# gogoex/BulletProofsPlus

Hardware: AMD Instinct MI355X
Metric: aggregated range-proof verifies/sec (n=64,m=16) (higher is better)
Workload: dtype u32 (30-bit limbs of a 381-bit prime field, v_mad_u64_u32)

## Files before the change

bulletproofsplus_amd/csrc/impl_verify.hpp:

```cpp
#pragma once
#include <functional>
#include <memory>
#include <mutex>

#include "codec.hpp"
#include "combined.hpp"
#include "fixed_launch.hpp"
#include "host_util.hpp"
#include "mixed.hpp"
#include "pippenger.hpp"

enum { BPP_STAGE_FROM_WIRE = 0, BPP_STAGE_SCALARS, BPP_STAGE_FIXED_MSM, BPP_STAGE_VAR_MSM, BPP_STAGE_FINALIZE,
       BPP_NUM_STAGES };
constexpr int BPP_PROFILE_SLOTS = 64;

namespace bpp {
struct PassShape {
    VerifyShape s;
    const uint32_t* challenges;
    TranscriptState tr0;
};
}

struct bpp_verifier {
    bpp_ctx ctx;
    bpp::VerifyShape s;
    bpp::DevBuf table;
    bpp::DevBuf challenges;
    bpp::TranscriptState tr0;
    std::vector<bpp::PassShape> views;
    bpp::DevBuf view_challenges;
    size_t table_bytes = 0;
    bool check_subgroup = false;
    bool profiling = false;
    std::vector<hipEvent_t> events;
    size_t passes_recorded = 0;
    unsigned last_blocks_per_proof = 0;
    unsigned last_horner_form = 0;
    hipStream_t aux = nullptr;
    hipEvent_t ev_fork = nullptr, ev_join = nullptr;
    std::mutex aux_mu;
    ~bpp_verifier() {
        for (hipEvent_t e : events) (void)hipEventDestroy(e);
        if (ev_fork) (void)hipEventDestroy(ev_fork);
        if (ev_join) (void)hipEventDestroy(ev_join);
        if (aux) (void)hipStreamDestroy(aux);
    }
};

namespace bpp {

inline unsigned blocks_per_proof(const VerifyShape& s, size_t count) {
    const unsigned maxb = cdiv(s.NF, FIXED_BLOCK);
    size_t tpp = ((size_t)1 << 18) / (count ? count : 1);
    tpp = std::max<size_t>(FIXED_BLOCK, std::min<size_t>(tpp, s.NF));
    const unsigned b_lat = cdiv(tpp, FIXED_BLOCK);
    const unsigned b_thr = std::min<unsigned>(cdiv((size_t)32768, count ? count : 1),
                                              std::max<unsigned>(1, s.NF / (FIXED_BLOCK * 4)));
#ifdef BPP_FORCE_PER
    if (count >= 1024) return std::max(1u, std::min<unsigned>(BPP_FORCE_PER, maxb));
#endif
    return std::max(1u, std::min(std::max(b_lat, b_thr), maxb));
}

#ifndef BPP_HORNER_TREE_MAX
#define BPP_HORNER_TREE_MAX 256
#endif
constexpr size_t HORNER_TREE_MAX = BPP_HORNER_TREE_MAX;
constexpr unsigned FOLD_GROUP = 8;
constexpr unsigned FOLD_GROUP2 = 4;

struct WsLayout {
    size_t pts, bad, scalars, prep, fthread, fpart, fpart2, fpart3, vpart, vdig, vwsum, vtbl, vscr, total;
};

template <class C>
struct VerifyImpl {
    static constexpr int N = C::Fp::N;
    static constexpr int JW = jac_words<C>();
    static constexpr int WW = 2 * N + 2;
    static constexpr int PW = WW / 2;

    static WsLayout ws_layout(const VerifyShape& s, size_t count) {
        WsLayout w;
        WsCarver o;
        w.pts = o.take(count * s.NV * 2 * N * 4);
        w.bad = o.take(count * 4);
        w.scalars = o.take(count * (size_t)s.N * 32);
        w.prep = o.take(count * vs_prep_bytes<C>(s));
        w.fthread = o.take(count * blocks_per_proof(s, count) * FIXED_BLOCK * JW * 4);
        w.fpart = o.take(count * blocks_per_proof(s, count) * (FIXED_BLOCK / FOLD_GROUP) * JW * 4);
        w.fpart2 = o.take(count * blocks_per_proof(s, count) * (FIXED_BLOCK / FOLD_GROUP / FOLD_GROUP2) * JW * 4);
        w.fpart3 = o.take(count * (FIXED_BLOCK / FOLD_GROUP / FOLD_GROUP2) * JW * 4);
        w.vpart = o.take(count * JW * 4);
        w.vdig = o.take(count * s.NV * VAR_DIGIT_STRIDE);
        w.vwsum = o.take(count * var_wsums_max<C>() * JW * 4);
        w.vtbl = o.take(count * s.NV * VAR_MULTIPLES * 2 * N * 4);
        w.vscr = o.take(count * s.NV * 2 * (VAR_MULTIPLES - 1) * N * 4);
        w.total = o.total;
        return w;
    }

    static int create(const bpp_ctx& ctx, const uint64_t* gh, const uint64_t* G, const uint64_t* H, size_t n, size_t m,
                      int window_bits, bpp_verifier** out);

    static PassShape own(const bpp_verifier* v) { return PassShape{v->s, v->challenges.u32(), v->tr0}; }
    static PassShape class_shape(const bpp_verifier* v, uint32_t c) {
        return c < v->views.size() ? v->views[c] : own(v);
    }

    static int run(bpp_verifier* v, const PassShape& ps, const uint64_t* d_points, const uint64_t* d_scalars, size_t count,
                   const uint64_t* d_challenges, uint32_t* d_ok, void* d_workspace, size_t workspace_bytes,
                   uint64_t* d_out_scalars, uint64_t* d_out_result, hipStream_t st);
    static int run(bpp_verifier* v, const uint64_t* d_points, const uint64_t* d_scalars, size_t count,
                   const uint64_t* d_challenges, uint32_t* d_ok, void* d_workspace, size_t workspace_bytes,
                   uint64_t* d_out_scalars, uint64_t* d_out_result, hipStream_t st) {
        return run(v, own(v), d_points, d_scalars, count, d_challenges, d_ok, d_workspace, workspace_bytes, d_out_scalars,
                   d_out_result, st);
    }

    static int range_scalars(const PassShape& ps, const uint64_t* d_scalars, const uint64_t* d_challenges, uint32_t* w_sc,
                             size_t count, uint32_t* w_prep, hipStream_t st) {
        const uint32_t* ch = d_challenges ? reinterpret_cast<const uint32_t*>(d_challenges) : ps.challenges;
        const uint32_t ch_stride = d_challenges ? (3 + ps.s.k) * 8 : 0;
        return launch_verify_scalars<C>(ps.s, reinterpret_cast<const uint32_t*>(d_scalars), ch, ch_stride, w_sc, count, w_prep, st);
    }

    using ScalarStage = std::function<int(uint32_t* w_sc, uint32_t* w_prep, uint32_t* w_bad, hipStream_t st)>;
    static int run_stage(bpp_verifier* v, const VerifyShape& s, const uint64_t* d_points, size_t count,
                         const ScalarStage& scalars, uint32_t* d_ok, void* d_workspace, size_t workspace_bytes,
                         uint64_t* d_out_scalars, uint64_t* d_out_result, hipStream_t st);

    static uint32_t horner_form(const VerifyShape& s, size_t count) {
        const bool small_job = (double)count * ((double)s.NF * fixed_adds_per_generator(s) / 7.0e9 + 9.2e-8) < 2.0e-3;
        return count <= HORNER_TREE_MAX ? 1u : (small_job ? 2u : 0u);
    }
    static int fork_tables(bpp_verifier* v, hipStream_t st, const uint32_t* w_pts, uint32_t* w_vt, uint32_t* w_vscr, size_t items,
                           std::unique_lock<std::mutex>& lock) {
        lock = std::unique_lock<std::mutex>(v->aux_mu);
        if (!v->aux) {
            HIPCHK(hipStreamCreateWithFlags(&v->aux, hipStreamNonBlocking));
            HIPCHK(hipEventCreateWithFlags(&v->ev_fork, hipEventDisableTiming));
            HIPCHK(hipEventCreateWithFlags(&v->ev_join, hipEventDisableTiming));
        }
        HIPCHK(hipEventRecord(v->ev_fork, st));
        HIPCHK(hipStreamWaitEvent(v->aux, v->ev_fork, 0));
        hipLaunchKernelGGL(k_var_tables<C>, dim3(cdiv(items, VAR_BLOCK)), dim3(VAR_BLOCK), 0, v->aux, w_pts, w_vt, w_vscr, items);
        HIPCHK(hipEventRecord(v->ev_join, v->aux));
        return BPP_OK;
    }
    static int join_tables(bpp_verifier* v, hipStream_t st, std::unique_lock<std::mutex>& lock) {
        HIPCHK(hipStreamWaitEvent(st, v->ev_join, 0));
        lock.unlock();
        return BPP_OK;
    }
    static hipError_t mark(hipEvent_t* ev, int idx, hipStream_t st) { return ev ? hipEventRecord(ev[idx], st) : hipSuccess; }
    template <class Layout>
    static int begin_pass(bpp_verifier* v, const PassShape& ps, const uint64_t* d_points, const uint64_t* d_scalars,
                          size_t count, const uint64_t* d_challenges, uint8_t* ws, const Layout& L, uint32_t* w_sc,
                          std::unique_lock<std::mutex>& aux_lock, hipStream_t st, hipEvent_t* ev);
    template <class Layout>
    static int begin_points(bpp_verifier* v, const VerifyShape& s, const uint64_t* d_points, size_t count, uint8_t* ws,
                            const Layout& L, std::unique_lock<std::mutex>& aux_lock, hipStream_t st, hipEvent_t* ev);
    template <class Layout, class FixedSums>
    static int weighted_windows(bpp_verifier* v, const PassShape& ps, uint8_t* ws, const Layout& L, size_t count,
                                const uint8_t* weight_key, uint64_t index_base, const uint64_t* d_weights, uint32_t per,
                                uint32_t split, std::unique_lock<std::mutex>& aux_lock, hipStream_t st,
                                FixedSums&& fixed_sums);
    template <class Layout>
    static int weighted_middle(bpp_verifier* v, const PassShape& ps, uint8_t* ws, const Layout& L, size_t count, uint32_t per,
                               uint32_t split, std::unique_lock<std::mutex>& aux_lock, hipStream_t st);
    static size_t fold_windows(const uint32_t* in, size_t nrem, uint32_t step, uint32_t* out, uint32_t per, hipStream_t st);
    static int finish(bpp_verifier* v, const VerifyShape& s, uint8_t* ws, const WsLayout& L, size_t count,
                      const uint32_t* w_sc, const uint32_t* w_vw, const uint32_t* w_bad, uint32_t* d_ok,
                      uint32_t* d_out_result, uint32_t tree, bool lone, hipStream_t st, hipEvent_t* ev);

    static int derive_challenges(bpp_verifier* v, const PassShape& ps, const uint64_t* d_points, size_t count,
                                 uint64_t* d_challenges, hipStream_t st);
    static int derive_challenges(bpp_verifier* v, const uint64_t* d_points, size_t count, uint64_t* d_challenges,
                                 hipStream_t st) {
        return derive_challenges(v, own(v), d_points, count, d_challenges, st);
    }

    struct MixedFront {
        size_t idx, pts, sc3, status, challenges, ok;
    };
    static MixedFront carve_front(WsCarver& o, const MixedPlan& p, size_t count, bool serialized) {
        MixedFront f;
        f.idx = o.take(count * (serialized ? (size_t)SX_WORDS : (size_t)MX_WORDS) * 4);
        f.pts = o.take(p.points * WW * 4);
        f.sc3 = o.take(count * 96);
        f.status = o.take(serialized ? count * 4 : 0);
        f.challenges = o.take(p.chals * 32);
        f.ok = o.take(count * 4);
        return f;
    }
    static int gather_front(const MixedPlan& p, const MixedFront& front, size_t count, const uint64_t* d_points,
                            const uint64_t* d_scalars, const uint64_t* d_challenges, uint8_t* ws, hipStream_t st);
    static int decode_front(const MixedPlan& p, const MixedFront& front, size_t count, const uint8_t* d_proofs,
                            const uint8_t* d_commitments, uint32_t version, uint8_t* ws, hipStream_t st);
    static int scatter_verdicts(const MixedFront& front, uint8_t* ws, uint32_t* d_ok, size_t count, hipStream_t st);
    struct ClassView {
        uint32_t c;
        PassShape ps;
        size_t first, count;
        uint64_t *pts, *sc3, *challenges;
    };
    template <class F>
    static int for_each_class(const bpp_verifier* v, const MixedPlan& p, const MixedFront& front, uint8_t* ws, F&& f) {
        auto U64 = [&](size_t off) { return reinterpret_cast<uint64_t*>(ws + off); };
        for (uint32_t c = 0; c < MIXED_CLASSES; c++) {
            if (!p.count[c]) continue;
            const int rc = f(ClassView{c, class_shape(v, c), p.first[c], p.count[c], U64(front.pts) + p.pt[c] * PW,
                                       U64(front.sc3) + p.first[c] * 12, U64(front.challenges) + p.chal[c] * 4});
            if (rc) return rc;
        }
// ... 324 lines not shown
        const uint32_t f1 = std::min<uint32_t>(s.NF, f0 + slab);
        const size_t total = (size_t)(f1 - f0) * runs_f;
        hipLaunchKernelGGL(k_tbl_fill<C>, dim3(cdiv(total, 64)), dim3(64), 0, nullptr, s, v->table.u32(),
                           tbl_scratch.u32(), f0, f1);
    }
    tr_initial_state<C>(s.n, s.m, reinterpret_cast<const uint32_t*>(fixed.data()), s.NF, v->tr0.st);
    std::vector<uint32_t> ch;
    default_challenges(s, ch);
    e = v->challenges.alloc(ch.size() * 4);
    if (e == hipSuccess) e = hipMemcpy(v->challenges.p, ch.data(), ch.size() * 4, hipMemcpyHostToDevice);
    std::vector<uint32_t> vch;
    std::vector<size_t> voff;
    for (uint32_t mp = 1; mp < s.m; mp <<= 1) {
        PassShape ps{};
        rc = make_verify_shape<C>(n, mp, window_bits, ps.s);
        if (rc) return rc;
        ps.s.hgap = s.n * (s.m - mp);
        std::vector<uint64_t> prefix((size_t)ps.s.NF * PW);
        std::memcpy(prefix.data(), fixed.data(), (size_t)(2 + ps.s.mn) * PW * 8);
        std::memcpy(prefix.data() + (size_t)(2 + ps.s.mn) * PW, fixed.data() + (size_t)(2 + s.mn) * PW,
                    (size_t)ps.s.mn * PW * 8);
        tr_initial_state<C>(ps.s.n, ps.s.m, reinterpret_cast<const uint32_t*>(prefix.data()), ps.s.NF, ps.tr0.st);
        std::vector<uint32_t> c1;
        default_challenges(ps.s, c1);
        voff.push_back(vch.size());
        vch.insert(vch.end(), c1.begin(), c1.end());
        v->views.push_back(ps);
    }
    if (e == hipSuccess && !vch.empty()) {
        e = v->view_challenges.alloc(vch.size() * 4);
        if (e == hipSuccess) e = hipMemcpy(v->view_challenges.p, vch.data(), vch.size() * 4, hipMemcpyHostToDevice);
        for (size_t i = 0; i < v->views.size(); i++) v->views[i].challenges = v->view_challenges.u32() + voff[i];
    }
    if (e == hipSuccess) e = hipDeviceSynchronize();
    if (e == hipSuccess) e = hipGetLastError();
    if (e != hipSuccess) return fail(BPP_E_HIP, "table build failed: ", hipGetErrorString(e));
    *out = v.release();
    return BPP_OK;
}

template <class C>
template <class Layout>
int VerifyImpl<C>::begin_points(bpp_verifier* v, const VerifyShape& s, const uint64_t* d_points, size_t count, uint8_t* ws,
                                const Layout& L, std::unique_lock<std::mutex>& aux_lock, hipStream_t st, hipEvent_t* ev) {
    uint32_t* w_pts = reinterpret_cast<uint32_t*>(ws + L.pts);
    uint32_t* w_bad = reinterpret_cast<uint32_t*>(ws + L.bad);
    const size_t npts = count * s.NV;
    HIPCHK(zero_words_async(w_bad, count * 4, st));
    HIPCHK(mark(ev, 2 * BPP_STAGE_FROM_WIRE, st));
    hipLaunchKernelGGL(k_points_from_wire<C>, dim3(cdiv(npts, 128)), dim3(128), 0, st,
                       reinterpret_cast<const uint32_t*>(d_points), w_pts, w_bad, npts, s.NV, v->check_subgroup ? 1u : 0u);
    HIPCHK(mark(ev, 2 * BPP_STAGE_FROM_WIRE + 1, st));
    return fork_tables(v, st, w_pts, reinterpret_cast<uint32_t*>(ws + L.vtbl), reinterpret_cast<uint32_t*>(ws + L.vscr), npts,
                       aux_lock);
}

template <class C>
template <class Layout>
int VerifyImpl<C>::begin_pass(bpp_verifier* v, const PassShape& ps, const uint64_t* d_points, const uint64_t* d_scalars,
                              size_t count, const uint64_t* d_challenges, uint8_t* ws, const Layout& L, uint32_t* w_sc,
                              std::unique_lock<std::mutex>& aux_lock, hipStream_t st, hipEvent_t* ev) {
    int rc = begin_points(v, ps.s, d_points, count, ws, L, aux_lock, st, ev);
    if (rc) return rc;
    HIPCHK(mark(ev, 2 * BPP_STAGE_SCALARS, st));
    rc = range_scalars(ps, d_scalars, d_challenges, w_sc, count, reinterpret_cast<uint32_t*>(ws + L.prep), st);
    if (rc) return rc;
    HIPCHK(mark(ev, 2 * BPP_STAGE_SCALARS + 1, st));
    return BPP_OK;
}

template <class C>
template <class Layout, class FixedSums>
int VerifyImpl<C>::weighted_windows(bpp_verifier* v, const PassShape& ps, uint8_t* ws, const Layout& L, size_t count,
                                    const uint8_t* weight_key, uint64_t index_base, const uint64_t* d_weights, uint32_t per,
                                    uint32_t split, std::unique_lock<std::mutex>& aux_lock, hipStream_t st,
                                    FixedSums&& fixed_sums) {
    uint32_t* w_wt = reinterpret_cast<uint32_t*>(ws + L.weights);
    WeightKey wk;
    load_key_words(d_weights ? nullptr : weight_key, wk.w);
    hipLaunchKernelGGL(k_comb_weights<C>, dim3(cdiv(count, 256)), dim3(256), 0, st, wk, index_base,
                       reinterpret_cast<const uint32_t*>(d_weights), w_wt, count);
    fixed_sums(w_wt);
    return weighted_middle(v, ps, ws, L, count, per, split, aux_lock, st);
}

template <class C>
template <class Layout>
int VerifyImpl<C>::weighted_middle(bpp_verifier* v, const PassShape& ps, uint8_t* ws, const Layout& L, size_t count,
                                   uint32_t per, uint32_t split, std::unique_lock<std::mutex>& aux_lock, hipStream_t st) {
    const VerifyShape& s = ps.s;
    auto W = [&](size_t off) { return reinterpret_cast<uint32_t*>(ws + off); };
    uint32_t *w_sc = W(L.scalars), *w_wt = W(L.weights), *w_vs = W(L.var_sc);
    uint8_t* w_vd = ws + L.vdig;
    const size_t items = count * s.NV;
    hipLaunchKernelGGL(k_comb_var_scalars<C>, dim3(cdiv(items, 256)), dim3(256), 0, st, s, w_sc, w_wt, w_vs, items);
    hipLaunchKernelGGL(k_var_digits<C>, dim3(cdiv(items, 256)), dim3(256), 0, st, s, w_vs, w_vd, items, 1u);
    int rc = join_tables(v, st, aux_lock);
    if (rc) return rc;
    const size_t vlanes = count * per;
    hipLaunchKernelGGL(k_var_windows<C>, dim3(cdiv(vlanes, VAR_BLOCK)), dim3(VAR_BLOCK), 0, st, s, w_vd, W(L.vtbl),
                       W(L.vwsum), vlanes, split, 1u);
    return BPP_OK;
}

template <class C>
size_t VerifyImpl<C>::fold_windows(const uint32_t* in, size_t nrem, uint32_t step, uint32_t* out, uint32_t per,
                                   hipStream_t st) {
    const size_t outn = cdiv(nrem, step);
    hipLaunchKernelGGL(k_comb_window_fold<C>, dim3(cdiv(outn * per, 64)), dim3(64), 0, st, in, nrem, step, out, outn * per,
                       per);
    return outn;
}

template <class C>
int VerifyImpl<C>::run(bpp_verifier* v, const PassShape& ps, const uint64_t* d_points, const uint64_t* d_scalars,
                       size_t count, const uint64_t* d_challenges, uint32_t* d_ok, void* d_workspace,
                       size_t workspace_bytes, uint64_t* d_out_scalars, uint64_t* d_out_result, hipStream_t st) {
    return run_stage(v, ps.s, d_points, count,
                     [&](uint32_t* w_sc, uint32_t* w_prep, uint32_t*, hipStream_t st_) {
                         return range_scalars(ps, d_scalars, d_challenges, w_sc, count, w_prep, st_);
                     },
                     d_ok, d_workspace, workspace_bytes, d_out_scalars, d_out_result, st);
}

template <class C>
int VerifyImpl<C>::run_stage(bpp_verifier* v, const VerifyShape& s, const uint64_t* d_points, size_t count,
                             const ScalarStage& scalars, uint32_t* d_ok, void* d_workspace, size_t workspace_bytes,
                             uint64_t* d_out_scalars, uint64_t* d_out_result, hipStream_t st) {
    const WsLayout L = ws_layout(s, count);
    if (workspace_bytes < L.total) return fail(BPP_E_ARG, "workspace too small");
    uint8_t* ws = static_cast<uint8_t*>(d_workspace);
    uint32_t* w_bad = reinterpret_cast<uint32_t*>(ws + L.bad);
    uint32_t* w_sc = d_out_scalars ? reinterpret_cast<uint32_t*>(d_out_scalars)
                                   : reinterpret_cast<uint32_t*>(ws + L.scalars);
    uint32_t* w_vt = reinterpret_cast<uint32_t*>(ws + L.vtbl);
    const unsigned bpp_ = blocks_per_proof(s, count);
    const size_t npts = count * s.NV;
    hipEvent_t* ev = nullptr;
    if (v->profiling) {
        ev = v->events.data() + (v->passes_recorded % BPP_PROFILE_SLOTS) * (BPP_NUM_STAGES * 2);
        v->passes_recorded++;
    }
    v->last_blocks_per_proof = bpp_;
    std::unique_lock<std::mutex> aux_lock;
    int rc = begin_points(v, s, d_points, count, ws, L, aux_lock, st, ev);
    if (rc) return rc;
    HIPCHK(mark(ev, 2 * BPP_STAGE_SCALARS, st));
    rc = scalars(w_sc, reinterpret_cast<uint32_t*>(ws + L.prep), w_bad, st);
    if (rc) return rc;
    HIPCHK(mark(ev, 2 * BPP_STAGE_SCALARS + 1, st));
    uint8_t* w_vd = ws + L.vdig;
    uint32_t* w_vw = reinterpret_cast<uint32_t*>(ws + L.vwsum);
    const uint32_t tree = horner_form(s, count);
    const bool lone = tree == 1 && count * bpp_ <= 1024;
    const uint32_t vgroups = lone ? VAR_GROUPS : 1u;
    v->last_horner_form = lone ? 3u : tree;
    const size_t vlanes = count * (tree == 1 ? var_wsums<C>() * vgroups : var_windows<C>());
    HIPCHK(mark(ev, 2 * BPP_STAGE_VAR_MSM, st));
    hipLaunchKernelGGL(k_var_digits<C>, dim3(cdiv(npts, 256)), dim3(256), 0, st, s, w_sc, w_vd, npts, 0u);
    rc = join_tables(v, st, aux_lock);
    if (rc) return rc;
    hipLaunchKernelGGL(k_var_windows<C>, dim3(cdiv(vlanes, VAR_BLOCK)), dim3(VAR_BLOCK), 0, st, s, w_vd, w_vt, w_vw,
                       vlanes, tree == 1 ? 1u : 0u, vgroups);
    HIPCHK(mark(ev, 2 * BPP_STAGE_VAR_MSM + 1, st));
    return finish(v, s, ws, L, count, w_sc, w_vw, w_bad, d_ok, reinterpret_cast<uint32_t*>(d_out_result), tree, lone, st,
                  ev);
}

template <class C>
int VerifyImpl<C>::finish(bpp_verifier* v, const VerifyShape& s, uint8_t* ws, const WsLayout& L, size_t count,
                          const uint32_t* w_sc, const uint32_t* w_vw, const uint32_t* w_bad, uint32_t* d_ok,
                          uint32_t* d_out_result, uint32_t tree, bool lone, hipStream_t st, hipEvent_t* ev) {
    const unsigned bpp_ = blocks_per_proof(s, count);
    uint32_t* w_fp = reinterpret_cast<uint32_t*>(ws + L.fpart);
    uint32_t* w_vp = reinterpret_cast<uint32_t*>(ws + L.vpart);
    HIPCHK(mark(ev, 2 * BPP_STAGE_FIXED_MSM, st));
    const unsigned hb = tree == 1 ? (unsigned)count : cdiv(count, tree == 2 ? FIXED_BLOCK / 8 : FIXED_BLOCK);
    uint32_t* w_ft = reinterpret_cast<uint32_t*>(ws + L.fthread);
    launch_fixed_msm<C, 0>((unsigned)(hb + count * bpp_), st, s, w_sc, v->table.u32(), w_ft, bpp_, hb, w_vw, w_vp, count,
                           lone ? 3u : tree, VpSel{1u, 0u, 1u, 0u});
    HIPCHK(mark(ev, 2 * BPP_STAGE_FIXED_MSM + 1, st));
    HIPCHK(mark(ev, 2 * BPP_STAGE_FINALIZE, st));
    const unsigned folded = bpp_ * (FIXED_BLOCK / FOLD_GROUP);
    const unsigned folded2 = folded / FOLD_GROUP2;
    uint32_t* w_fp2 = reinterpret_cast<uint32_t*>(ws + L.fpart2);
    if (tree == 1) {
        if (!lone)
            hipLaunchKernelGGL(k_partials_fold<C>, dim3(cdiv(count * folded, 64)), dim3(64), 0, st, w_ft, FOLD_GROUP, w_fp,
                               count * folded);
        hipLaunchKernelGGL(k_finalize_tree<C>, dim3((unsigned)count), dim3(64), 0, st, lone ? w_ft : w_fp,
                           lone ? bpp_ : folded, w_vp, w_bad, d_ok, d_out_result, count);
        HIPCHK(mark(ev, 2 * BPP_STAGE_FINALIZE + 1, st));
        HIPCHK(hipGetLastError());
        return BPP_OK;
    }
    hipLaunchKernelGGL(k_partials_fold<C>, dim3(cdiv(count * folded, 64)), dim3(64), 0, st, w_ft, FOLD_GROUP, w_fp,
                       count * folded);
    hipLaunchKernelGGL(k_partials_fold<C>, dim3(cdiv(count * folded2, 64)), dim3(64), 0, st, w_fp, FOLD_GROUP2, w_fp2,
                       count * folded2);
    const uint32_t* w_last = w_fp2;
    unsigned last = folded2;
    if (bpp_ > 1) {
        uint32_t* w_fp3 = reinterpret_cast<uint32_t*>(ws + L.fpart3);
        last = folded2 / bpp_;
        hipLaunchKernelGGL(k_partials_fold<C>, dim3(cdiv(count * last, 64)), dim3(64), 0, st, w_fp2, bpp_, w_fp3,
                           count * last);
        w_last = w_fp3;
    }
    hipLaunchKernelGGL(k_finalize<C>, dim3(cdiv(count, 64)), dim3(64), 0, st, w_last, last, w_vp, 1u, w_bad, d_ok,
                       d_out_result, count);
    HIPCHK(mark(ev, 2 * BPP_STAGE_FINALIZE + 1, st));
    HIPCHK(hipGetLastError());
    return BPP_OK;
}

template <class C>
int VerifyImpl<C>::run_serialized(bpp_verifier* v, const uint8_t* d_proofs, const uint8_t* d_commitments, size_t count,
                                  bool transcript, uint32_t* d_ok, void* d_workspace, size_t workspace_bytes,
                                  hipStream_t st, uint32_t version, const GroupedArgs* grouped) {
    const VerifyShape& s = v->s;
    if (int rc = container_args_ok(v, version)) return rc;
    const SerLayout L = ser_layout(s, count, grouped ? grouped->group : 0u);
    if (workspace_bytes < L.total) return fail(BPP_E_ARG, "workspace too small");
    uint8_t* ws = static_cast<uint8_t*>(d_workspace);
    uint32_t* w_rec = reinterpret_cast<uint32_t*>(ws + L.records);
    uint32_t* w_sc = reinterpret_cast<uint32_t*>(ws + L.scalars);
    uint32_t* w_st = reinterpret_cast<uint32_t*>(ws + L.status);
    uint64_t* w_ch = reinterpret_cast<uint64_t*>(ws + L.challenges);
    HIPCHK(zero_words_async(w_st, count * 4, st));
    hipLaunchKernelGGL(k_container_decode<C>, dim3(cdiv(count * s.NV, 64)), dim3(64), 0, st, s, d_proofs, d_commitments,
                       w_rec, w_sc, w_st, count, version);
    if constexpr (C::ID == 0)
        hipLaunchKernelGGL(k_records_subgroup<C>, dim3(cdiv(count * s.NV, 64)), dim3(64), 0, st, w_rec, w_st, s.NV,
                           count * s.NV);
    HIPCHK(hipGetLastError());
    if (transcript) {
        int rc = derive_challenges(v, reinterpret_cast<const uint64_t*>(w_rec), count, w_ch, st);
        if (rc) return rc;
    }
    int rc = grouped ? run_grouped(v, reinterpret_cast<const uint64_t*>(w_rec), reinterpret_cast<const uint64_t*>(w_sc), count,
                                   transcript ? w_ch : nullptr, grouped->weight_key, grouped->index_base, grouped->d_weights,
                                   grouped->group, d_ok, grouped->h_stats, ws + L.run, workspace_bytes - L.run, st)
                     : run(v, reinterpret_cast<const uint64_t*>(w_rec), reinterpret_cast<const uint64_t*>(w_sc), count,
                           transcript ? w_ch : nullptr, d_ok, ws + L.run, workspace_bytes - L.run, nullptr, nullptr, st);
    if (rc) return rc;
    hipLaunchKernelGGL(k_container_status<C>, dim3(cdiv(count, 256)), dim3(256), 0, st, w_st, d_ok, count);
    HIPCHK(hipGetLastError());
    return BPP_OK;
}

template <class C>
int VerifyImpl<C>::derive_challenges(bpp_verifier* v, const PassShape& ps, const uint64_t* d_points, size_t count,
                                     uint64_t* d_challenges, hipStream_t st) {
    (void)v;
    hipLaunchKernelGGL(k_transcript_challenges<C>, dim3(cdiv(count, 64)), dim3(64), 0, st, ps.s, ps.tr0,
                       reinterpret_cast<const uint32_t*>(d_points), reinterpret_cast<uint32_t*>(d_challenges), count);
    HIPCHK(hipGetLastError());
    return BPP_OK;
}

template <class C>
int VerifyImpl<C>::gather_front(const MixedPlan& p, const MixedFront& front, size_t count, const uint64_t* d_points,
                                const uint64_t* d_scalars, const uint64_t* d_challenges, uint8_t* ws, hipStream_t st) {
    auto U64 = [&](size_t off) { return reinterpret_cast<uint64_t*>(ws + off); };
    uint32_t* w_idx = reinterpret_cast<uint32_t*>(ws + front.idx);
    HIPCHK(hipMemcpyAsync(w_idx, p.idx.data(), p.idx.size() * 4, hipMemcpyHostToDevice, st));
    hipLaunchKernelGGL(k_mixed_gather<C>, dim3((unsigned)count), dim3(MIXED_BLOCK), 0, st, w_idx, count, d_points, d_scalars,
                       d_challenges, U64(front.pts), U64(front.sc3), U64(front.challenges));
    HIPCHK(hipGetLastError());
    return BPP_OK;
}

template <class C>
int VerifyImpl<C>::decode_front(const MixedPlan& p, const MixedFront& front, size_t count, const uint8_t* d_proofs,
                                const uint8_t* d_commitments, uint32_t version, uint8_t* ws, hipStream_t st) {
    auto W = [&](size_t off) { return reinterpret_cast<uint32_t*>(ws + off); };
    uint32_t *w_idx = W(front.idx), *w_rec = W(front.pts), *w_st = W(front.status);
    HIPCHK(hipMemcpyAsync(w_idx, p.sidx.data(), p.sidx.size() * 4, hipMemcpyHostToDevice, st));
    HIPCHK(zero_words_async(w_st, count * 4, st));
    const unsigned waves = (unsigned)(p.lanes / SER_WAVE);
    hipLaunchKernelGGL(k_container_decode_mixed<C>, dim3(waves), dim3(SER_WAVE), 0, st, p.classes, w_idx, d_proofs,
                       d_commitments, w_rec, W(front.sc3), w_st, version);
    if constexpr (C::ID == 0)
        hipLaunchKernelGGL(k_records_subgroup_mixed<C>, dim3(waves), dim3(SER_WAVE), 0, st, p.classes, w_rec, w_st);
    HIPCHK(hipGetLastError());
    return BPP_OK;
}

template <class C>
int VerifyImpl<C>::scatter_verdicts(const MixedFront& front, uint8_t* ws, uint32_t* d_ok, size_t count, hipStream_t st) {
    auto W = [&](size_t off) { return reinterpret_cast<const uint32_t*>(ws + off); };
    hipLaunchKernelGGL(k_mixed_status_scatter<C>, dim3(cdiv(count, 256)), dim3(256), 0, st, W(front.idx), W(front.status),
                       W(front.ok), d_ok, count);
    HIPCHK(hipGetLastError());
    return BPP_OK;
}

template <class C>
int VerifyImpl<C>::run_mixed(bpp_verifier* v, const uint64_t* d_points, const uint64_t* d_scalars, const uint32_t* m_of,
                             size_t count, const uint64_t* d_challenges, uint32_t* d_ok, void* d_workspace,
                             size_t workspace_bytes, uint64_t* d_out_result, hipStream_t st) {
    MixedPlan p;
    int rc = mixed_plan(v->s, m_of, count, true, p);
    if (rc) return rc;
    const MixedLayout L = mixed_layout(v, p, count);
    if (workspace_bytes < L.total) return fail(BPP_E_ARG, "workspace too small");
    uint8_t* ws = static_cast<uint8_t*>(d_workspace);
    rc = gather_front(p, L.f, count, d_points, d_scalars, d_challenges, ws, st);
    if (rc) return rc;
    uint32_t* w_ok = reinterpret_cast<uint32_t*>(ws + L.f.ok);
    uint64_t* w_res = d_out_result ? reinterpret_cast<uint64_t*>(ws + L.result) : nullptr;
    rc = for_each_class(v, p, L.f, ws, [&](const ClassView& cv) {
        return run(v, cv.ps, cv.pts, cv.sc3, cv.count, d_challenges ? cv.challenges : nullptr, w_ok + cv.first, ws + L.run,
                   workspace_bytes - L.run, nullptr, w_res ? w_res + cv.first * PW : nullptr, st);
    });
    if (rc) return rc;
    hipLaunchKernelGGL(k_mixed_scatter<C>, dim3(cdiv(count, 4)), dim3(256), 0, st,
                       reinterpret_cast<const uint32_t*>(ws + L.f.idx), count, w_ok, w_res, nullptr, d_ok, d_out_result,
                       nullptr);
    HIPCHK(hipGetLastError());
    return BPP_OK;
}

template <class C>
int VerifyImpl<C>::derive_challenges_mixed(bpp_verifier* v, const uint64_t* d_points, const uint32_t* m_of, size_t count,
                                           uint64_t* d_challenges, void* d_workspace, size_t workspace_bytes,
                                           hipStream_t st) {
    MixedPlan p;
    int rc = mixed_plan(v->s, m_of, count, true, p);
    if (rc) return rc;
    const MixedLayout L = mixed_layout(v, p, count);
    if (workspace_bytes < L.total) return fail(BPP_E_ARG, "workspace too small");
    uint8_t* ws = static_cast<uint8_t*>(d_workspace);
    rc = gather_front(p, L.f, count, d_points, nullptr, nullptr, ws, st);
    if (rc) return rc;
    rc = for_each_class(v, p, L.f, ws, [&](const ClassView& cv) {
        return derive_challenges(v, cv.ps, cv.pts, cv.count, cv.challenges, st);
    });
    if (rc) return rc;
    hipLaunchKernelGGL(k_mixed_scatter<C>, dim3(cdiv(count, 4)), dim3(256), 0, st,
                       reinterpret_cast<const uint32_t*>(ws + L.f.idx), count, nullptr, nullptr,
                       reinterpret_cast<uint64_t*>(ws + L.f.challenges), nullptr, nullptr, d_challenges);
    HIPCHK(hipGetLastError());
    return BPP_OK;
}

template <class C>
int VerifyImpl<C>::run_serialized_mixed(bpp_verifier* v, const uint8_t* d_proofs, const uint8_t* d_commitments,
                                        const uint32_t* m_of, size_t count, bool transcript, uint32_t* d_ok,
                                        void* d_workspace, size_t workspace_bytes, hipStream_t st, uint32_t version) {
    if (int rc = container_args_ok(v, version)) return rc;
    MixedPlan p;
    int rc = mixed_plan_serialized(v->s, m_of, count, (size_t)container_point_bytes<C>(version), true, p);
    if (rc) return rc;
    const SerMixedLayout L = ser_mixed_layout(v, p, count);
    if (workspace_bytes < L.total) return fail(BPP_E_ARG, "workspace too small");
    uint8_t* ws = static_cast<uint8_t*>(d_workspace);
    auto W = [&](size_t off) { return reinterpret_cast<uint32_t*>(ws + off); };
    rc = decode_front(p, L.f, count, d_proofs, d_commitments, version, ws, st);
// ... 389 lines not shown
```

bulletproofsplus_amd/csrc/kernels.hpp:

```cpp
#pragma once
#include <hip/hip_runtime.h>
#include "ec.hpp"
#include "fixed_glv.hpp"
#include "ed25519.hpp"
#include "ristretto.hpp"
#include "transcript.hpp"

namespace bpp {

constexpr unsigned MSM_BLOCK = 64;
constexpr unsigned VS_PB = 8;
constexpr unsigned VS_BLOCK = VS_PB * 64;
constexpr unsigned FIXED_BLOCK = 128;
constexpr unsigned VAR_BLOCK = 64;
template <class C>
constexpr bool var_glv() {
    return curve_has_glv<C>();
}
template <class C>
constexpr uint32_t var_windows() {
    return var_glv<C>() ? 33u : 65u;
}
template <class C>
constexpr uint32_t var_wsums() {
    return var_windows<C>() * (var_glv<C>() ? 2u : 1u);
}
constexpr uint32_t VAR_GROUPS = 3;
template <class C>
constexpr uint32_t var_wsums_max() {
    return var_wsums<C>() * VAR_GROUPS;
}
constexpr uint32_t VAR_DIGIT_STRIDE = 80;
constexpr uint32_t VAR_MULTIPLES = 8;
#ifndef BPP_FIXED_WAVES
#define BPP_FIXED_WAVES 2
#endif
#ifndef BPP_VAR_WAVES
#define BPP_VAR_WAVES 2
#endif
#ifndef BPP_VAR_TABLES_WAVES
#define BPP_VAR_TABLES_WAVES 2
#endif


static __global__ void __launch_bounds__(256) k_zero_words(uint32_t* __restrict__ p, size_t words) {
    const size_t i = (size_t)blockIdx.x * blockDim.x + threadIdx.x;
    if (i < words) p[i] = 0;
}
inline hipError_t zero_words_async(void* p, size_t bytes, hipStream_t st) {
    const size_t words = (bytes + 3) / 4;
    if (words == 0) return hipSuccess;
    hipLaunchKernelGGL(k_zero_words, dim3((unsigned)((words + 255) / 256)), dim3(256), 0, st, static_cast<uint32_t*>(p), words);
    return hipGetLastError();
}

template <int NW>
__device__ __forceinline__ void ld_words(const uint32_t* __restrict__ p, uint32_t* dst) {
    static_assert(NW % 4 == 0, "16-byte granules");
    const uint4* q = reinterpret_cast<const uint4*>(p);
#pragma unroll
    for (int i = 0; i < NW / 4; i++) {
        uint4 v = q[i];
        dst[4 * i] = v.x;
        dst[4 * i + 1] = v.y;
        dst[4 * i + 2] = v.z;
        dst[4 * i + 3] = v.w;
    }
}
template <int NW>
__device__ __forceinline__ void st_words(uint32_t* __restrict__ p, const uint32_t* src) {
    static_assert(NW % 4 == 0, "16-byte granules");
    uint4* q = reinterpret_cast<uint4*>(p);
#pragma unroll
    for (int i = 0; i < NW / 4; i++) q[i] = make_uint4(src[4 * i], src[4 * i + 1], src[4 * i + 2], src[4 * i + 3]);
}

template <class C>
__device__ __forceinline__ Aff<C> aff_ldg(const uint32_t* __restrict__ p) {
    constexpr int N = C::Fp::N;
    constexpr int JW = jac_words<C>();
    uint32_t w[2 * N];
    ld_words<2 * N>(p, w);
    return aff_load<C>(w);
}
template <class C>
__device__ __forceinline__ void aff_stg(uint32_t* __restrict__ p, const Aff<C>& a) {
    constexpr int N = C::Fp::N;
    constexpr int JW = jac_words<C>();
    uint32_t w[2 * N];
    aff_store(a, w);
    st_words<2 * N>(p, w);
}
template <class C>
__device__ __forceinline__ Jac<C> jac_ldg(const uint32_t* __restrict__ p) {
    constexpr int N = C::Fp::N;
    constexpr int JW = jac_words<C>();
    uint32_t w[JW];
    ld_words<JW>(p, w);
    return jac_load<C>(w);
}
template <class C>
__device__ __forceinline__ void jac_stg(uint32_t* __restrict__ p, const Jac<C>& a) {
    constexpr int N = C::Fp::N;
    constexpr int JW = jac_words<C>();
    uint32_t w[JW];
    jac_store(a, w);
    st_words<JW>(p, w);
}

template <class C>
__device__ __forceinline__ Jac<C> block_reduce_jac(Jac<C> acc, uint32_t* lds) {
    constexpr int N = C::Fp::N;
    constexpr int JW = jac_words<C>();
    const int tid = threadIdx.x;
    for (int half = blockDim.x >> 1; half >= 1; half >>= 1) {
        if (tid >= half && tid < 2 * half) jac_store(acc, lds + (size_t)tid * JW);
        __syncthreads();
        if (tid < half) acc = jac_add(acc, jac_load<C>(lds + (size_t)(tid + half) * JW));
        __syncthreads();
    }
    return acc;
}

template <class T>
__device__ __forceinline__ T wave_shfl(const T& v, int src_lane) {
    static_assert(sizeof(T) % 4 == 0, "whole words");
    struct Words {
        uint32_t w[sizeof(T) / 4];
    };
    Words a = __builtin_bit_cast(Words, v);
#pragma unroll
    for (int i = 0; i < (int)(sizeof(T) / 4); i++) a.w[i] = (uint32_t)__shfl((int)a.w[i], src_lane, 64);
    return __builtin_bit_cast(T, a);
}

template <class C>
__device__ __forceinline__ Jac<C> wave_sum_jac(Jac<C> x, int span = 64) {
    const int lane = threadIdx.x & 63;
#pragma unroll 1
    for (int d = span >> 1; d >= 1; d >>= 1) {
        const Jac<C> o = wave_shfl(x, lane ^ d);
        x = jac_add(x, o);
    }
    return x;
}

template <class C>
__device__ __forceinline__ Jac<C> jac_dbl_tri(const Jac<C>& p) {
    using F = Fe<typename C::Fp>;
    static_assert(C::ID != 2, "short-Weierstrass curves");
    const int lane = threadIdx.x & 63;
    const int role = lane % 3, g0 = lane - role;
    auto pick = [](bool c, const F& a, const F& b) {
        F r;
#pragma unroll
        for (int i = 0; i < C::Fp::NL; i++) r.l[i] = c ? a.l[i] : b.l[i];
        return r;
    };
    const F m1 = fe_mul(pick(role == 0, p.X, p.Y), pick(role == 0, p.X, pick(role == 1, p.Y, p.Z)));
    const F B = wave_shfl(m1, (g0 + 1) & 63);
    const F m2 = fe_sqr(pick(role == 0, fe_add(fe_dbl(m1), m1), pick(role == 1, m1, fe_add(p.X, B))));
    const F A = wave_shfl(m1, g0), Fq = wave_shfl(m2, g0), Cc = wave_shfl(m2, (g0 + 1) & 63);
    const F t = wave_shfl(m2, (g0 + 2) & 63), YZ = wave_shfl(m1, (g0 + 2) & 63);
    const F D = fe_dbl(fe_sub(fe_sub(t, A), Cc));
    const F E = fe_add(fe_dbl(A), A);
    Jac<C> r;
// ... 563 lines not shown
        j++;
    }
    const uint32_t d0 = r * TBL_RUN + 1;
    const uint32_t n = min(TBL_RUN, cnt - (d0 - 1));
    uint32_t* win = table + ((size_t)f * s.per_f + s.went[j]) * 2 * N;
    const Aff<C> base = aff_ldg<C>(win);
    Jac<C> J;
    if (d0 == 1) {
        J = jac_from_aff(base);
    } else {
        uint32_t kw[1] = {d0};
        J = aff_mul_words(base, kw, 1);
    }
    affine_chain<C>(J, win, n, win + (size_t)(d0 - 1) * 2 * N, scratch + idx * 2 * TBL_RUN * N);
}


template <class C, bool SPLIT>
__device__ __forceinline__ Jac<C> var_wsum_ld(const uint32_t* __restrict__ wsum, size_t b, uint32_t j, uint32_t groups = 1) {
    constexpr int JW = jac_words<C>();
    constexpr uint32_t NW = var_windows<C>();
    const uint32_t parts = SPLIT ? (var_wsums<C>() / NW) * groups : 1u;
    const uint32_t* W = wsum + b * parts * NW * JW;
    Jac<C> sj = jac_ldg<C>(W + (size_t)j * JW);
    for (uint32_t t = 1; t < parts; t++) sj = jac_add(sj, jac_ldg<C>(W + (size_t)(t * NW + j) * JW));
    return sj;
}

template <class C>
__device__ __forceinline__ void var_horner_lane(const uint32_t* __restrict__ wsum, uint32_t* __restrict__ out, size_t b) {
    constexpr int JW = jac_words<C>();
    constexpr uint32_t NW = var_windows<C>();
    Jac<C> acc = var_wsum_ld<C, false>(wsum, b, NW - 1);
    for (int j = (int)NW - 2; j >= 0; j--) {
        if (!acc.is_inf()) {
            acc = jac_dbl(acc);
            acc = jac_dbl(acc);
            acc = jac_dbl(acc);
            acc = jac_dbl(acc);
        }
        acc = jac_add(acc, var_wsum_ld<C, false>(wsum, b, (uint32_t)j));
    }
    jac_stg<C>(out + b * JW, acc);
}

template <class C>
__device__ __forceinline__ void var_horner_wave2(const uint32_t* __restrict__ wsum, uint32_t* __restrict__ out, size_t b,
                                                 uint32_t* lds, uint32_t groups) {
    constexpr uint32_t NW = var_windows<C>(), PER = 21;
    static_assert(NW <= 2 * PER, "two waves hold the windows");
    constexpr int JW = jac_words<C>();
    const uint32_t wave = threadIdx.x >> 6, lane = threadIdx.x & 63u;
    const uint32_t q = lane / 3, j = wave * PER + q;
    const bool has = q < PER && j < NW;
    Jac<C> R = has ? var_wsum_ld<C, true>(wsum, b, j, groups) : jac_inf<C>();
    const uint32_t times = has ? 4 * j : 0u;
    const uint32_t maxt = 4 * (wave == 0 ? PER - 1 : NW - 1);
    for (uint32_t t = 0; t < maxt; t++) {
        const Jac<C> d = jac_dbl_tri<C>(R);
        if (t < times) R = d;
    }
    R = wave_shfl(R, (int)((3 * lane) & 63u));
    if (lane >= PER || wave * PER + lane >= NW) R = jac_inf<C>();
    R = wave_sum_jac<C>(R, 32);
    if (wave == 1 && lane == 0) jac_store(R, lds);
    __syncthreads();
    if (wave == 0 && lane == 0) jac_stg<C>(out + b * JW, jac_add(R, jac_load<C>(lds)));
}

__device__ __forceinline__ void var_horner_wave_ed(const uint32_t* __restrict__ wsum, uint32_t* __restrict__ out, size_t b,
                                                   uint32_t groups) {
    using C = Ed25519;
    constexpr uint32_t NW = var_windows<C>();
    static_assert(NW == 65, "sixteen quads x four windows + one");
    constexpr int JW = jac_words<C>();
    const uint32_t lane = threadIdx.x & 63u, q = lane >> 2;
    Jac<C> acc = jac_inf<C>();
    if (q == 0) {
        acc = var_wsum_ld<C, true>(wsum, b, 64, groups);
        for (int t = 0; t < 64; t++) acc = ed_dbl_quad(acc);
    }
    for (int w = 3; w >= 0; w--) {
        acc = jac_add(acc, var_wsum_ld<C, true>(wsum, b, q + 16 * (uint32_t)w, groups));
        const int times = w > 0 ? 64 : 60;
        for (int t = 0; t < times; t++) {
            const Jac<C> d = ed_dbl_quad(acc);
            if (w > 0 || (uint32_t)t < 4 * q) acc = d;
        }
    }
    acc = wave_shfl(acc, (int)((4 * lane) & 63u));
    if (lane >= 16) acc = jac_inf<C>();
    acc = wave_sum_jac<C>(acc, 16);
    if (lane == 0) jac_stg<C>(out + b * JW, acc);
}

template <class C>
__device__ __forceinline__ void var_horner_group(const uint32_t* __restrict__ wsum, uint32_t* __restrict__ out, size_t b,
                                                 bool active, uint32_t* lds_wave) {
    constexpr uint32_t NW = var_windows<C>(), L = NW - 1, G = 8, CW = L / G;
    static_assert(L % G == 0, "windows split evenly over the eight lanes");
    constexpr int JW = jac_words<C>();
    const uint32_t lane = threadIdx.x & 63u, g = lane & (G - 1);
    Jac<C> acc = jac_inf<C>();
    if (active) {
        const int lo = (int)(g * CW);
        const int top = g == G - 1 ? (int)L : lo + (int)CW - 1;
        acc = var_wsum_ld<C, false>(wsum, b, (uint32_t)top);
        for (int j = top - 1; j >= lo; j--) {
            if (!acc.is_inf()) {
                acc = jac_dbl(acc);
                acc = jac_dbl(acc);
                acc = jac_dbl(acc);
                acc = jac_dbl(acc);
            }
            acc = jac_add(acc, var_wsum_ld<C, false>(wsum, b, (uint32_t)j));
        }
    }
    for (uint32_t stride = 1; stride < G; stride <<= 1) {
        jac_store(acc, lds_wave + (size_t)lane * JW);
        __builtin_amdgcn_fence(__ATOMIC_SEQ_CST, "wavefront");
        __builtin_amdgcn_wave_barrier();
        if (active && (g & (2 * stride - 1)) == 0) {
            Jac<C> hi = jac_load<C>(lds_wave + (size_t)(lane + stride) * JW);
            if (!hi.is_inf())
                for (uint32_t t = 0; t < 4 * CW * stride; t++) hi = jac_dbl(hi);
            acc = jac_add(acc, hi);
        }
        __builtin_amdgcn_fence(__ATOMIC_SEQ_CST, "wavefront");
        __builtin_amdgcn_wave_barrier();
    }
    if (active && g == 0) jac_stg<C>(out + b * JW, acc);
}

__device__ __forceinline__ void glds16(const uint32_t* gsrc, uint32_t lds_byte_addr) {
    unsigned keep;
    lds_byte_addr = __builtin_amdgcn_readfirstlane(lds_byte_addr);
    asm volatile("s_mov_b32 %0, m0\n\ts_mov_b32 m0, %2\n\ts_nop 0\n\tglobal_load_lds_dwordx4 %1, off\n\ts_mov_b32 m0, %0"
                 : "=&s"(keep)
                 : "v"(gsrc), "s"(lds_byte_addr)
                 : "memory");
}

#ifndef BPP_FIXED_RING
#define BPP_FIXED_RING 2
#endif
constexpr int FIXED_RING = BPP_FIXED_RING;
template <class C>
constexpr unsigned fixed_lds_bytes() {
    return (FIXED_BLOCK / 64) * (FIXED_RING * (2 * C::Fp::N / 4) + 2) * 1024;
}

struct VpSel {
    uint32_t nvp, first, cnt, prover;
};

template <class C>
constexpr int fixed_waves() {
    return C::Fp::NL > 9 ? BPP_FIXED_WAVES : 3;
}
template <class C, int ROLE = 0>
__global__ void __launch_bounds__(FIXED_BLOCK, fixed_waves<C>()) k_fixed_msm(VerifyShape s, const uint32_t* __restrict__ scalars,
                            const uint32_t* __restrict__ table, uint32_t* __restrict__ partials, uint32_t per,
                            uint32_t horner_blocks, const uint32_t* __restrict__ wsum, uint32_t* __restrict__ var_out,
                            size_t horner_count, uint32_t horner_tree, VpSel sel) {
    constexpr int N = C::Fp::N;
    constexpr int JW = jac_words<C>();
    constexpr int CH = 2 * N / 4;
    constexpr int WAVE_WORDS = (FIXED_RING * CH + 2) * 256;
    constexpr bool GLV = fixed_glv<C>();
    constexpr int NWD = GLV ? GLV_HALF_WORDS : WIN_FULL_WORDS;
    extern __shared__ __align__(16) uint32_t lds[];
    if (blockIdx.x < horner_blocks) {
        if (horner_tree == 2) {
            const size_t b = (size_t)blockIdx.x * (blockDim.x / 8) + threadIdx.x / 8;
            var_horner_group<C>(wsum, var_out, b, b < horner_count, lds + (size_t)(threadIdx.x >> 6) * 64 * JW);
        } else if (horner_tree) {
            const size_t b = blockIdx.x;
            if constexpr (var_glv<C>()) {
                if (b < horner_count) var_horner_wave2<C>(wsum, var_out, b, lds, horner_tree == 3 ? VAR_GROUPS : 1u);
            } else {
                if (b < horner_count && threadIdx.x < 64) var_horner_wave_ed(wsum, var_out, b, horner_tree == 3 ? VAR_GROUPS : 1u);
            }
        } else {
            const size_t lane = (size_t)blockIdx.x * blockDim.x + threadIdx.x;
            if (lane < horner_count) var_horner_lane<C>(wsum, var_out, lane);
        }
        return;
    }
#ifdef BPP_XCD_REMAP
    uint32_t bid = blockIdx.x - horner_blocks;
    {
        const uint32_t nb = gridDim.x - horner_blocks;
        if (nb % 8 == 0 && horner_blocks % 8 == 0) bid = (bid % 8) * (nb / 8) + bid / 8;
    }
#else
    const uint32_t bid = blockIdx.x - horner_blocks;
#endif
    const size_t b = bid / per;
    const uint32_t part = bid % per;
    const uint32_t* sc = scalars + ((b / sel.cnt) * sel.nvp + sel.first + b % sel.cnt) * (size_t)s.N * 8;
    const uint32_t stride = per * blockDim.x;
    const uint32_t lane = threadIdx.x & 63u;
    uint32_t* ring = lds + (threadIdx.x >> 6) * WAVE_WORDS;
    uint32_t* sbuf = ring + FIXED_RING * CH * 256;
    const uint32_t ring_addr = (uint32_t)reinterpret_cast<uintptr_t>(ring);
    const uint32_t sbuf_addr = ring_addr + FIXED_RING * CH * 1024;
    const uint32_t f0 = part * blockDim.x + threadIdx.x;
    const uint32_t first = part * blockDim.x;
    uint32_t NFc = s.NF, cmode = 0, cbit = 0, neg_from = 0xffffffffu;
    if (sel.prover) {
        const uint32_t vp = sel.first + (uint32_t)(b % sel.cnt);
        if (vp == 0) {
            neg_from = 2 + s.mn;
        } else if (vp <= 2 * s.k) {
            cmode = 1 + ((vp - 1) & 1u);
            cbit = s.k - 1 - (vp - 1) / 2;
            NFc = 2 + s.mn;
        } else if (vp >= 2 * s.k + 3) {
            NFc = 2;
        }
    }
    auto gen_of = [&](uint32_t x) -> uint32_t {
        if (cmode == 0 || x < 2) return x;
        uint32_t u = x - 2;
        const uint32_t hm = s.mn >> 1;
        const bool isH = u >= hm;
        if (isH) u -= hm;
        const uint32_t bitv = ((cmode == 1) != isH) ? 1u : 0u;
        const uint32_t j = ((u >> cbit) << (cbit + 1)) | (bitv << cbit) | (u & ((1u << cbit) - 1u));
        return 2 + (isH ? s.mn : 0u) + j;
    };
    const bool spread = NFc >= stride;
    const uint32_t G = spread ? NFc / stride : (first < NFc ? 1u : 0u);
    const uint32_t T = G * s.W;
    constexpr uint32_t PH = GLV ? 2u : 1u;
    const uint32_t LWH = spread ? (NFc - G * stride) * s.W : 0u;
    const uint32_t LW = PH * LWH;
    const uint32_t TT = T + (LW + stride - 1) / stride;
    const uint32_t NQ = PH * G;
    Xyzz<C> acc = xyzz_inf<C>();

    auto dma_scalar = [&](uint32_t g) {
        const uint32_t x = f0 + g * stride;
        const uint32_t* src = x < NFc ? sc + (size_t)fixed_term_index(s, gen_of(x)) * 8 : sc;
        asm volatile("s_waitcnt lgkmcnt(0)" ::: "memory");
        glds16(src, sbuf_addr);
        glds16(src + 4, sbuf_addr + 1024);
    };
    uint32_t w[NWD];
    uint32_t hneg = 0;
    uint32_t pi = 0;
    auto take = [&](const uint32_t* v, uint32_t which, uint32_t* out, uint32_t& negate) {
        if constexpr (GLV) {
            uint32_t k1[4], k2[4];
            bool n1, n2;
            glv_split_balanced<C>(v, k1, k2, n1, n2);
            win_biased<NWD>(which ? k1 : k2, s.bias, out);
            negate = which ? (n1 ? 1u : 0u) : (n2 ? 0u : 1u);
        } else {
            win_biased<NWD>(v, s.bias, out);
            negate = 0;
        }
    };
    auto take_scalar = [&]() {
        const uint4* q = reinterpret_cast<const uint4*>(sbuf);
        const uint4 lo = q[lane], hi = q[64 + lane];
        const uint32_t v[8] = {lo.x, lo.y, lo.z, lo.w, hi.x, hi.y, hi.z, hi.w};
        take(v, pi, w, hneg);
    };
    auto window = [&](uint32_t j, uint32_t& cj, uint32_t& e0) {
        if constexpr (GLV) {
            cj = win_width(s, j);
            e0 = s.went[j];
        } else {
            cj = j + 1 < s.W ? s.c : 0u;
            e0 = j << (s.c - 1);
        }
    };
    uint32_t ti = 0, gi = 0, ji = 0;
    uint32_t vbits = 0, nbits = 0;
    uint32_t bbits = 0;
    auto issue = [&]() {
        const uint32_t slot = (GLV ? pi * T + ti : ti) % FIXED_RING;
        const uint32_t* src = table;
        uint32_t valid = 0, neg = 0, viabeta = 0;
        auto entry = [&](int32_t dg, uint32_t f, uint32_t e0, uint32_t hn) {
            const uint32_t mag = dg < 0 ? (uint32_t)(-dg) : (uint32_t)dg;
            src = table + ((size_t)table_generator(s, f) * s.per_f + e0 + (mag - 1)) * 2 * N;
            valid = 1;
            neg = (dg < 0 ? 1u : 0u) ^ hn ^ (f >= neg_from ? 1u : 0u);
        };
        if (ti < T) {
            const uint32_t qi = pi * G + gi;
            if (ji == 0 && qi > 0) {
                take_scalar();
                if (qi + 1 < NQ) dma_scalar(gi + 1 < G ? gi + 1 : 0u);
            }
            const uint32_t x = f0 + gi * stride;
            uint32_t cj, e0;
            window(ji, cj, e0);
            const int32_t dg = win_next_digit(w, cj);
            if (x < NFc && dg != 0) entry(dg, gen_of(x), e0, hneg);
        } else if (pi + 1 == PH && ti < TT) {
            const uint32_t x = (ti - T) * stride + f0;
            if (x < LW) {
                const uint32_t which = x >= LWH ? 1u : 0u, xh = x - which * LWH;
                const uint32_t l = xh / s.W, jx = xh - l * s.W;
                const uint32_t f = gen_of(G * stride + l);
                uint32_t v[8], we[NWD], hn;
                ld_words<8>(sc + (size_t)fixed_term_index(s, f) * 8, v);
                take(v, which, we, hn);
                if constexpr (GLV) viabeta = 1u - which;
                int32_t dg = 0;
                uint32_t e0 = 0;
                for (uint32_t r = 0; r < s.W; r++) {
                    uint32_t cr, er;
                    window(r, cr, er);
                    const int32_t d = win_next_digit(we, cr);
                    if (r == jx) {
                        dg = d;
                        e0 = er;
                    }
                }
                if (dg != 0) entry(dg, f, e0, hn);
            }
        }
        asm volatile("s_waitcnt lgkmcnt(0)" ::: "memory");
#pragma unroll
        for (int k = 0; k < CH; k++) glds16(src + 4 * k, ring_addr + (slot * CH + k) * 1024);
        vbits = (vbits & ~(1u << slot)) | (valid << slot);
        nbits = (nbits & ~(1u << slot)) | (neg << slot);
        if constexpr (GLV) bbits = (bbits & ~(1u << slot)) | (viabeta << slot);
        ti++;
        if (++ji == s.W) {
            ji = 0;
            gi++;
        }
        if constexpr (GLV) {
            if (ti == T && pi == 0) {
                pi = 1;
                ti = 0;
                gi = 0;
                ji = 0;
            }
        }
    };
    if (G) {
        dma_scalar(0);
        asm volatile("s_waitcnt vmcnt(0)" ::: "memory");
        take_scalar();
        if (NQ > 1) dma_scalar(G > 1 ? 1u : 0u);
    }
    for (int d = 0; d < FIXED_RING; d++) issue();
// ... 231 lines not shown
```

Measured before the change: 202,100.

## Split fixed-base MSM into single-block long proofs plus multi-block tail proofs

Result: faster. 206,200 (median of 6 runs) (+2.1%).

```diff
diff --git a/bulletproofsplus_amd/csrc/fixed_plan.hpp b/bulletproofsplus_amd/csrc/fixed_plan.hpp
--- /dev/null
+++ b/bulletproofsplus_amd/csrc/fixed_plan.hpp
@@ -0,0 +1,60 @@
+#pragma once
+#include <stddef.h>
+#include <stdint.h>
+
+#include <algorithm>
+
+#include "field.hpp"
+
+namespace bpp {
+
+constexpr unsigned FIXED_BLOCK = 128;
+
+constexpr size_t FIXED_RESIDENT = 1024;
+#ifndef BPP_FIXED_SHORT_PROOFS
+#define BPP_FIXED_SHORT_PROOFS FIXED_RESIDENT
+#endif
+
+inline unsigned blocks_per_proof(uint32_t NF, size_t count) {
+    const unsigned maxb = (NF + FIXED_BLOCK - 1) / FIXED_BLOCK;
+    size_t tpp = ((size_t)1 << 18) / (count ? count : 1);
+    tpp = std::max<size_t>(FIXED_BLOCK, std::min<size_t>(tpp, NF));
+    const unsigned b_lat = (unsigned)((tpp + FIXED_BLOCK - 1) / FIXED_BLOCK);
+    const unsigned b_thr = std::min<unsigned>((unsigned)((32 * FIXED_RESIDENT + (count ? count : 1) - 1) / (count ? count : 1)),
+                                              std::max<unsigned>(1, NF / (FIXED_BLOCK * 4)));
+#ifdef BPP_FORCE_PER
+    if (count >= FIXED_RESIDENT) return std::max(1u, std::min<unsigned>(BPP_FORCE_PER, maxb));
+#endif
+    return std::max(1u, std::min(std::max(b_lat, b_thr), maxb));
+}
+
+struct FixedPlan {
+    unsigned per;
+    size_t long_count;
+};
+
+inline FixedPlan fixed_plan(uint32_t NF, size_t count, uint32_t horner_form) {
+    FixedPlan p{blocks_per_proof(NF, count), 0};
+    const size_t short_proofs = (size_t)(BPP_FIXED_SHORT_PROOFS);
+    if (horner_form == 0 && count > FIXED_RESIDENT && count > short_proofs && NF / (FIXED_BLOCK * 4) >= 2 && p.per >= 2)
+        p.long_count = count - short_proofs;
+    return p;
+}
+
+inline size_t fixed_plan_blocks(const FixedPlan& p, size_t count) { return p.long_count + (count - p.long_count) * p.per; }
+
+BPP_HD void fixed_block_of(uint32_t bid, uint32_t per, uint32_t long_count, uint32_t& proof, uint32_t& part,
+                           uint32_t& per_here) {
+    if (bid < long_count) {
+        proof = bid;
+        part = 0;
+        per_here = 1;
+    } else {
+        const uint32_t r = bid - long_count;
+        proof = long_count + r / per;
+        part = r % per;
+        per_here = per;
+    }
+}
+
+}
diff --git a/bulletproofsplus_amd/csrc/impl_verify.hpp b/bulletproofsplus_amd/csrc/impl_verify.hpp
--- a/bulletproofsplus_amd/csrc/impl_verify.hpp
+++ b/bulletproofsplus_amd/csrc/impl_verify.hpp
@@ -50,18 +50,7 @@
 
 namespace bpp {
 
-inline unsigned blocks_per_proof(const VerifyShape& s, size_t count) {
-    const unsigned maxb = cdiv(s.NF, FIXED_BLOCK);
-    size_t tpp = ((size_t)1 << 18) / (count ? count : 1);
-    tpp = std::max<size_t>(FIXED_BLOCK, std::min<size_t>(tpp, s.NF));
-    const unsigned b_lat = cdiv(tpp, FIXED_BLOCK);
-    const unsigned b_thr = std::min<unsigned>(cdiv((size_t)32768, count ? count : 1),
-                                              std::max<unsigned>(1, s.NF / (FIXED_BLOCK * 4)));
-#ifdef BPP_FORCE_PER
-    if (count >= 1024) return std::max(1u, std::min<unsigned>(BPP_FORCE_PER, maxb));
-#endif
-    return std::max(1u, std::min(std::max(b_lat, b_thr), maxb));
-}
+inline unsigned blocks_per_proof(const VerifyShape& s, size_t count) { return blocks_per_proof(s.NF, count); }
 
 #ifndef BPP_HORNER_TREE_MAX
 #define BPP_HORNER_TREE_MAX 256
@@ -692,7 +681,7 @@
     uint8_t* w_vd = ws + L.vdig;
     uint32_t* w_vw = reinterpret_cast<uint32_t*>(ws + L.vwsum);
     const uint32_t tree = horner_form(s, count);
-    const bool lone = tree == 1 && count * bpp_ <= 1024;
+    const bool lone = tree == 1 && count * bpp_ <= FIXED_RESIDENT;
     const uint32_t vgroups = lone ? VAR_GROUPS : 1u;
     v->last_horner_form = lone ? 3u : tree;
     const size_t vlanes = count * (tree == 1 ? var_wsums<C>() * vgroups : var_windows<C>());
@@ -711,18 +700,20 @@
 int VerifyImpl<C>::finish(bpp_verifier* v, const VerifyShape& s, uint8_t* ws, const WsLayout& L, size_t count,
                           const uint32_t* w_sc, const uint32_t* w_vw, const uint32_t* w_bad, uint32_t* d_ok,
                           uint32_t* d_out_result, uint32_t tree, bool lone, hipStream_t st, hipEvent_t* ev) {
-    const unsigned bpp_ = blocks_per_proof(s, count);
+    const FixedPlan plan = fixed_plan(s.NF, count, lone ? 3u : tree);
+    const unsigned bpp_ = plan.per;
+    const size_t longs = plan.long_count, shorts = count - longs, nblk = fixed_plan_blocks(plan, count);
     uint32_t* w_fp = reinterpret_cast<uint32_t*>(ws + L.fpart);
     uint32_t* w_vp = reinterpret_cast<uint32_t*>(ws + L.vpart);
     HIPCHK(mark(ev, 2 * BPP_STAGE_FIXED_MSM, st));
     const unsigned hb = tree == 1 ? (unsigned)count : cdiv(count, tree == 2 ? FIXED_BLOCK / 8 : FIXED_BLOCK);
     uint32_t* w_ft = reinterpret_cast<uint32_t*>(ws + L.fthread);
-    launch_fixed_msm<C, 0>((unsigned)(hb + count * bpp_), st, s, w_sc, v->table.u32(), w_ft, bpp_, hb, w_vw, w_vp, count,
-                           lone ? 3u : tree, VpSel{1u, 0u, 1u, 0u});
+    launch_fixed_msm<C, 0>((unsigned)(hb + nblk), st, s, w_sc, v->table.u32(), w_ft, bpp_, hb, w_vw, w_vp, count,
+                           lone ? 3u : tree, VpSel{1u, 0u, 1u, 0u, (uint32_t)longs});
     HIPCHK(mark(ev, 2 * BPP_STAGE_FIXED_MSM + 1, st));
     HIPCHK(mark(ev, 2 * BPP_STAGE_FINALIZE, st));
-    const unsigned folded = bpp_ * (FIXED_BLOCK / FOLD_GROUP);
-    const unsigned folded2 = folded / FOLD_GROUP2;
+    constexpr unsigned folded1 = FIXED_BLOCK / FOLD_GROUP, per_block = folded1 / FOLD_GROUP2;
+    const unsigned folded = bpp_ * folded1;
     uint32_t* w_fp2 = reinterpret_cast<uint32_t*>(ws + L.fpart2);
     if (tree == 1) {
         if (!lone)
@@ -734,17 +725,19 @@
         HIPCHK(hipGetLastError());
         return BPP_OK;
     }
-    hipLaunchKernelGGL(k_partials_fold<C>, dim3(cdiv(count * folded, 64)), dim3(64), 0, st, w_ft, FOLD_GROUP, w_fp,
-                       count * folded);
-    hipLaunchKernelGGL(k_partials_fold<C>, dim3(cdiv(count * folded2, 64)), dim3(64), 0, st, w_fp, FOLD_GROUP2, w_fp2,
-                       count * folded2);
+    hipLaunchKernelGGL(k_partials_fold<C>, dim3(cdiv(nblk * folded1, 64)), dim3(64), 0, st, w_ft, FOLD_GROUP, w_fp,
+                       nblk * folded1);
+    uint32_t* w_fp3 = reinterpret_cast<uint32_t*>(ws + L.fpart3);
+    if (longs)
+        hipLaunchKernelGGL(k_partials_fold<C>, dim3(cdiv(longs * per_block, 64)), dim3(64), 0, st, w_fp, FOLD_GROUP2, w_fp3,
+                           longs * per_block);
+    hipLaunchKernelGGL(k_partials_fold<C>, dim3(cdiv(shorts * bpp_ * per_block, 64)), dim3(64), 0, st,
+                       w_fp + longs * folded1 * JW, FOLD_GROUP2, w_fp2, shorts * bpp_ * per_block);
     const uint32_t* w_last = w_fp2;
-    unsigned last = folded2;
+    const unsigned last = per_block;
     if (bpp_ > 1) {
-        uint32_t* w_fp3 = reinterpret_cast<uint32_t*>(ws + L.fpart3);
-        last = folded2 / bpp_;
-        hipLaunchKernelGGL(k_partials_fold<C>, dim3(cdiv(count * last, 64)), dim3(64), 0, st, w_fp2, bpp_, w_fp3,
-                           count * last);
+        hipLaunchKernelGGL(k_partials_fold<C>, dim3(cdiv(shorts * last, 64)), dim3(64), 0, st, w_fp2, bpp_,
+                           w_fp3 + longs * last * JW, shorts * last);
         w_last = w_fp3;
     }
     hipLaunchKernelGGL(k_finalize<C>, dim3(cdiv(count, 64)), dim3(64), 0, st, w_last, last, w_vp, 1u, w_bad, d_ok,
diff --git a/bulletproofsplus_amd/csrc/kernels.hpp b/bulletproofsplus_amd/csrc/kernels.hpp
--- a/bulletproofsplus_amd/csrc/kernels.hpp
+++ b/bulletproofsplus_amd/csrc/kernels.hpp
@@ -2,6 +2,7 @@
 #include <hip/hip_runtime.h>
 #include "ec.hpp"
 #include "fixed_glv.hpp"
+#include "fixed_plan.hpp"
 #include "ed25519.hpp"
 #include "ristretto.hpp"
 #include "transcript.hpp"
@@ -11,7 +12,6 @@
 constexpr unsigned MSM_BLOCK = 64;
 constexpr unsigned VS_PB = 8;
 constexpr unsigned VS_BLOCK = VS_PB * 64;
-constexpr unsigned FIXED_BLOCK = 128;
 constexpr unsigned VAR_BLOCK = 64;
 template <class C>
 constexpr bool var_glv() {
@@ -881,6 +881,7 @@
 
 struct VpSel {
     uint32_t nvp, first, cnt, prover;
+    uint32_t long_count = 0;
 };
 
 template <class C>
@@ -920,14 +921,15 @@
     uint32_t bid = blockIdx.x - horner_blocks;
     {
         const uint32_t nb = gridDim.x - horner_blocks;
-        if (nb % 8 == 0 && horner_blocks % 8 == 0) bid = (bid % 8) * (nb / 8) + bid / 8;
+        if (sel.long_count == 0 && nb % 8 == 0 && horner_blocks % 8 == 0) bid = (bid % 8) * (nb / 8) + bid / 8;
     }
 #else
     const uint32_t bid = blockIdx.x - horner_blocks;
 #endif
-    const size_t b = bid / per;
-    const uint32_t part = bid % per;
-    const uint32_t* sc = scalars + ((b / sel.cnt) * sel.nvp + sel.first + b % sel.cnt) * (size_t)s.N * 8;
+    uint32_t b, part, per_here;
+    fixed_block_of(bid, per, sel.long_count, b, part, per_here);
+    per = per_here;
+    const uint32_t* sc = scalars + ((size_t)(b / sel.cnt) * sel.nvp + sel.first + b % sel.cnt) * (size_t)s.N * 8;
     const uint32_t stride = per * blockDim.x;
     const uint32_t lane = threadIdx.x & 63u;
     uint32_t* ring = lds + (threadIdx.x >> 6) * WAVE_WORDS;
```
